# team-attention/nobs-whisper

Hardware: AMD Instinct MI355X
Metric: audio-sec/s (RTF⁻¹) large-v3 greedy, batch 128; 1/2/4/8 MI355X (higher is better)
Workload: dtype bf16

## Files before the change

### include/whisper_mi355x.h

```cpp
#ifndef WHISPER_MI355X_H
#define WHISPER_MI355X_H

#include "whisper.h"

#ifdef __cplusplus
extern "C" {
#endif

#define WHISPER_MI355X_ERR_RUNTIME (-10)

enum whisper_mi355x_dtype { WHISPER_MI355X_F16 = 0, WHISPER_MI355X_BF16 = 1, WHISPER_MI355X_FP8_ENC = 2 };

WHISPER_API struct whisper_context * whisper_mi355x_init(const char * path_model, struct whisper_context_params params,
                                                         int dtype, bool load_weights);

WHISPER_API int whisper_mi355x_weight_arena(struct whisper_context * ctx, void ** dev_ptr, size_t * bytes);

WHISPER_API int whisper_mi355x_rccl_unique_id(char out[128]);
WHISPER_API int whisper_mi355x_broadcast_weights(struct whisper_context * ctx, const char unique_id[128], int rank, int world);

WHISPER_API int whisper_mi355x_full_batch(struct whisper_context * ctx, struct whisper_state * state,
                                          struct whisper_full_params params, const float * const * pcm,
                                          const int * n_samples, int n_jobs, bool pcm_on_device, int fixed_tokens);
WHISPER_API int whisper_mi355x_full_batch_forced(struct whisper_context * ctx, struct whisper_state * state,
// ... 42 lines not shown

WHISPER_API int whisper_mi355x_kernel_timing(struct whisper_state * state, int class_mask);
WHISPER_API int whisper_mi355x_kernel_stats(struct whisper_state * state, int cls, double out[3]);
#define WHISPER_MI355X_KSTAT_PDEC_GIVE_UPS 100
WHISPER_API long whisper_mi355x_pdec_give_ups(struct whisper_state * state);
#define WHISPER_MI355X_KSTAT_BEAM_GATHER 101

WHISPER_API int whisper_mi355x_debug_gemm(struct whisper_context * ctx, int epi, const void * A, int M, int K,
                                          const void * B, int N, const float * bias, void * out, int reps, float * ms);
WHISPER_API void whisper_mi355x_set_gemm_variant(int variant);
WHISPER_API void whisper_mi355x_set_gemm_stamps(void * dev);
WHISPER_API int whisper_mi355x_debug_gemm_small(struct whisper_context * ctx, int epi, const void * A, int M, int K,
                                                const void * B, int N, const float * bias, void * out,
                                                const float * ln_w, const float * ln_b, int reps, float * ms);
WHISPER_API void whisper_mi355x_set_dec_splits(int splits);
WHISPER_API void whisper_mi355x_set_dec_bm(int rows);
WHISPER_API void whisper_mi355x_set_pdec_spin(long ticks);
WHISPER_API void whisper_mi355x_set_pdec_stamps(void * dev);
WHISPER_API void whisper_mi355x_set_pdec_blocks(int on);
WHISPER_API int whisper_mi355x_debug_gemm_fp8(struct whisper_context * ctx, int epi, const void * A8,
                                              const float * a_scale, int M, int K, const void * B8,
                                              const float * b_scale, int N, const float * bias, void * out,
                                              int reps, float * ms);
WHISPER_API int whisper_mi355x_debug_gemm_w8(struct whisper_context * ctx, int epi, const void * A, int M, int K,
                                             const void * B8, const float * b_scale, int N, const float * bias,
                                             void * out, const float * ln_w, const float * ln_b, void * y);
WHISPER_API int whisper_mi355x_debug_quant_fp8(struct whisper_context * ctx, const void * x, long rows, int K,
                                               void * q, float * s);
WHISPER_API int whisper_mi355x_debug_attn_encoder(struct whisper_context * ctx, const void * qkv, int B, int T, int d,
                                                  int H, int variant, void * out, int reps, float * ms);
WHISPER_API int whisper_mi355x_debug_gemm_ln(struct whisper_context * ctx, const void * A, int M, int K,
                                             const void * B, int N, const float * bias, float * x,
                                             const float * ln_w, const float * ln_b, void * y, int reps, float * ms);

WHISPER_API int whisper_mi355x_debug_xattn(struct whisper_context * ctx, const void * enc, const int * slot,
                                           const void * q, const void * wkt, const void * wv, const float * bv,
                                           int n, int n_ctx, int d, float scale, int splits, float rescale_thr,
                                           void * out, int reps, float * ms);

WHISPER_API int whisper_mi355x_debug_attn_self_step(struct whisper_context * ctx, const float * slabs, int splits,
                                                    const float * bias, float scale, void * cache, const int * slot,
                                                    const int * pos, int n, int L, int layer, int H, int n_ctx,
                                                    void * out);
WHISPER_API int whisper_mi355x_debug_attn_cross_step(struct whisper_context * ctx, const float * slabs, int splits,
                                                     const float * bias, float scale, const void * cache,
                                                     const int * slot, const int * n_kv, int n, int L, int layer,
                                                     int H, int n_ctx, void * out);
WHISPER_API int whisper_mi355x_debug_attn_prefill(struct whisper_context * ctx, const void * q, int q_stride,
                                                  const void * cache, const int * slot, const int * n_kv,
                                                  const void * tiles, int n_tiles, int L, int layer, int H, int n_ctx,
                                                  void * out);

struct whisper_mi355x_cand {
    int32_t id, tid;
    float   p, plog, pt, ptsum, no_speech_prob, pad;
};
WHISPER_API int whisper_mi355x_debug_logits_topk(struct whisper_context * ctx, const float * logits, int n,
                                                 const int * rules, const float * temperature, int k, int split,
                                                 struct whisper_mi355x_cand * cand, struct whisper_mi355x_cand * greedy);
WHISPER_API int whisper_mi355x_debug_kv_gather(struct whisper_context * ctx, void * cache, int n_slots, int L, int H,
                                               int n_ctx, const int * copies, int n_copies, int * n_staged);

struct whisper_mi355x_seq_ctl {
    int32_t is_initial, last_ts, penult_ts, has_ts, seek_delta;
    float   temperature;
    int32_t suppress_blank, no_timestamps, suppress_eot, tid0_initial;
// ... 46 lines not shown
```

### nobs-whisper_amd/csrc/capi.cpp

```cpp
#include <cmath>
#include <cstring>
#include <string>
#include <thread>
#include <vector>

#include <rccl/rccl.h>

#include "../../include/whisper_mi355x.h"
#include "engine.h"

namespace wm { extern int g_gemm_variant; extern int g_dec_splits; extern int g_dec_bm; extern unsigned long long* g_gemm_stamps; }
using namespace wm;

static Context* C(whisper_context* ctx) { return ctx ? &ctx->c : nullptr; }

template <typename F> static int guarded(whisper_state* s, F&& f) {
    try {
        return f();
    } catch (const wm::Error&) {
    } catch (const std::bad_alloc&) {
        fprintf(stderr, "whisper_mi355x: host out of memory\n");
    }
    if (s) recover_state(s);
    return WHISPER_MI355X_ERR_RUNTIME;
// ... 743 lines not shown
int whisper_mi355x_debug_gemm_ln(struct whisper_context* ctx, const void* A, int M, int K, const void* B, int N,
                                 const float* bias, float* x, const float* ln_w, const float* ln_b, void* y, int reps,
                                 float* ms) {
    return guarded(nullptr, [&]() -> int {
        if (!ctx || M > 128) return -1;
        hipSetDevice(ctx->c.device);
        hipStream_t st;
        WM_CHECK(hipStreamCreate(&st));
        GemmArgs g{};
        g.A = A; g.a_rpb = M; g.a_bstride = 0; g.a_rstride = K;
        g.B = B; g.bias = bias; g.M = M; g.N = N; g.K = K;
        g.out = x; g.ldo = N; g.o_rpb = M; g.o_bstride = 0; g.o_off = 0;
        g.sc_div = 0; g.sc_mod = 1; g.sc_lim = 0; g.scale = 1.0f;
        g.ln_w = ln_w; g.ln_b = ln_b; g.ln_out = y;
        g.splitk_ws_elems = 64L * M * N;
        WM_CHECK(hipMalloc(&g.splitk_ws, g.splitk_ws_elems * sizeof(float)));
        hipEvent_t e0, e1;
        WM_CHECK(hipEventCreate(&e0));
        WM_CHECK(hipEventCreate(&e1));
        WM_CHECK(hipEventRecord(e0, st));
        for (int r = 0; r < std::max(1, reps); r++) launch_gemm(ctx->c.dt, EPI_RESID, g, st);
        WM_CHECK(hipEventRecord(e1, st));
        WM_CHECK(hipStreamSynchronize(st));
        float t = 0;
        WM_CHECK(hipEventElapsedTime(&t, e0, e1));
        if (ms) *ms = t / std::max(1, reps);
        hipEventDestroy(e0);
        hipEventDestroy(e1);
        hipStreamDestroy(st);
        hipFree(g.splitk_ws);
        return 0;
    });
}
int whisper_mi355x_debug_xattn(struct whisper_context* ctx, const void* enc, const int* slot, const void* q,
                               const void* wkt, const void* wv, const float* bv, int n, int n_ctx, int d, float scale,
                               int splits, float rescale_thr, void* out, int reps, float* ms) {
    return guarded(nullptr, [&]() -> int {
        if (!ctx || n <= 0 || !xattn_supported(d)) return -1;
        hipSetDevice(ctx->c.device);
        const DType dt = ctx->c.dt;
        const int H = d / 64;
        if (splits <= 0) splits = xattn_splits(n, n_ctx);
        void* qx = nullptr;
        float *op = nullptr, *ml = nullptr;
        WM_CHECK(hipMalloc(&qx, (size_t)n * 2 * H * d * 2));
        WM_CHECK(hipMalloc((void**)&op, (size_t)n * splits * H * d * 4));
        WM_CHECK(hipMalloc((void**)&ml, (size_t)n * splits * H * 2 * 4));
        hipStream_t st;
        WM_CHECK(hipStreamCreate(&st));
        auto run = [&] {
            launch_xattn_qproj(dt, q, wkt, n, d, H, scale, qx, st);
            launch_xattn_step(dt, enc, slot, qx, n, n_ctx, d, splits, rescale_thr, op, ml, st);
            launch_xattn_combine(dt, op, ml, splits, wv, bv, n, d, H, out, st);
        };
        hipEvent_t e0, e1;
        WM_CHECK(hipEventCreate(&e0));
        WM_CHECK(hipEventCreate(&e1));
        run();
        WM_CHECK(hipEventRecord(e0, st));
        for (int r = 0; r < reps; r++) run();
        WM_CHECK(hipEventRecord(e1, st));
        WM_CHECK(hipStreamSynchronize(st));
        float t = 0;
        WM_CHECK(hipEventElapsedTime(&t, e0, e1));
        if (ms) *ms = reps > 0 ? t / reps : 0.0f;
        hipEventDestroy(e0);
// ... 330 lines not shown
```

### nobs-whisper_amd/csrc/engine.cpp

```cpp
#include <algorithm>
#include <chrono>
#include <cmath>
#include <cstring>
#include <exception>
#include <thread>

#include "engine.h"

namespace wm {

static size_t esize(DType) { return 2; }

static void dfree(void*& p) {
    if (p) { void* q = p; p = nullptr; WM_CHECK(hipFree(q)); }
}
template <typename T> static void dfree(T*& p) {
    void* q = (void*)p;
    p = nullptr;
    dfree(q);
}
template <typename T> static void dalloc(T*& p, size_t bytes) {
    void* q = nullptr;
    p = nullptr;
    WM_CHECK(hipMalloc(&q, bytes));
// ... 705 lines not shown
    w.n_qtiles = nt;
    WM_CHECK(hipMemcpyAsync(w.qtiles, w.h_qtiles, (size_t)nt * sizeof(int2), hipMemcpyHostToDevice, s->stream));
}

struct DecView {
    int r0, n;
    hipStream_t st;
    float* splitk;
    long splitk_elems;
    float *xo, *xml;
};

static int small_m_max() {
    const char* e = getenv("WHISPER_MI355X_SMALLM");
    if (!e) return 4;
    const int v = atoi(e);
    return v == 1 ? 32 : std::max(0, std::min(32, v));
}

static int quant_small_max() {
    const char* e = getenv("WHISPER_MI355X_QSMALL_MAX");
    return e ? atoi(e) : 32;
}

static int pdec_max() {
    const char* e = getenv("WHISPER_MI355X_PDEC");
    return e ? std::max(0, std::min(kPdecMaxRows, atoi(e))) : kPdecMaxRows;
}

static int small_rows_max(Context* c) { return c->quant ? std::max(quant_small_max(), small_m_max()) : small_m_max(); }

static bool dec_fp8(Context* c) { return c->fp8_enc && !c->dec8.empty(); }

static int dec_path_sig() {
    return small_m_max() | (std::min(std::max(quant_small_max(), 0), 1023) << 6) |
           (std::min(std::max(attn_cross_wide_max(), 0), 1023) << 16) | (pdec_max() << 26) | ((g_pdec_blocks & 1) << 29);
}

static bool pdec_blocks(Context* c) {
    return c->quant && (g_pdec_blocks || !c->expanded.load(std::memory_order_acquire));
}

static bool pdec_use(Context* c, whisper_state* s, int n, bool xdirect) {
    if (xdirect || s->pdec_off || s->split_slots || n < 1 || n > pdec_max()) return false;
    if (dec_fp8(c)) return false;
    const bool quant = c->w.dec[0].qqkv.type != 0;
    for (const LayerW& L : c->w.dec)
        for (const QMat* q : {&L.qqkv, &L.qo, &L.qxq, &L.qxo, &L.q1, &L.q2})
            if ((q->type != 0) != quant) return false;
    const bool blocks = pdec_blocks(c);
    if (blocks && c->dt != DType::F16) return false;
    if (!pdec_supported(c->hp.n_text_state, c->hp.n_text_head, blocks)) return false;
    static const int cus = [] {
        int dev = 0, v = 0;
        hipGetDevice(&dev);
        hipDeviceGetAttribute(&v, hipDeviceAttributeMultiprocessorCount, dev);
        return v;
    }();
    return cus == 256;
}

static int dec_groups(int n_tok) { return cdiv(n_tok, 128); }

enum StepPath { STEP_PDEC, STEP_SMALL, STEP_SPLITK };
struct StepPlan {
    int n;
    int groups, gsz;
    StepPath path, tail_path;
    bool xdirect;
// ... 207 lines not shown
    const Hparams& hp = c->hp;
    Workspace& w = s->ws;
    const int d = hp.n_text_state, H = hp.n_text_head, V = hp.n_vocab, L = hp.n_text_layer;
    const DType dt = c->dt;
    const Weights& W = c->w;
    hipStream_t st = v.st;
    const int n = v.n;
    const DecRows r = dec_rows(c, s, v);
    const int KCLS = K_GEMM_DEC;
    const double kvrow = (double)H * 64 * 2 * 2;
    const int kt_stride = kt_layer_stride(s);
    auto gemm = [&](int epi, const GemmArgs& g) { tgemm_ws(s, KCLS, dt, epi, g, st, v.splitk, v.splitk_elems); };
    auto use8 = [&](GemmArgs g, void* q8, float* sc) {
        if (P.w8) { g.B = q8; g.w8_scale = sc; }
        return g;
    };
    auto resid = [&](const void* A, int K, const void* Wt, const float* bias, const float* lnw, const float* lnb, void* q8,
                     float* sc) {
        GemmArgs g = use8(gemm_plain(A, n, K, Wt, d, bias, r.dx, d), q8, sc);
        g.ln_w = lnw; g.ln_b = lnb; g.ln_out = r.dh;
        gemm(EPI_RESID, g);
    };
    auto partials = [&](const void* A, const void* Wt, int N, const float* bias, float scale, void* q8,
                        float* sc) -> DecSlabs {
        GemmArgs g = use8(gemm_plain(A, n, d, Wt, N, bias, nullptr, N), q8, sc);
        g.splitk_ws = v.splitk;
        g.splitk_ws_elems = v.splitk_elems;
        g.slab_wt = 1;
        KT kt(s, KCLS, 2.0 * g.N * g.K + 2.0 * g.M * g.K + 4.0 * g.M * g.N, st);
        const int splits = launch_gemm_partials(dt, g, st);
        if (splits <= 0 || splits > 16) WM_FAIL("decode partials GEMM not applicable (splits %d)", splits);
        return DecSlabs{v.splitk, splits, (long)n * N, N, bias, scale};
    };
    embed_rows(c, r, true);
    for (int l = 0; l < L; l++) {
        const LayerW Lw = layer_dense(c, s, l, st);
        static const Context::Fp8Dec no8{};
        const Context::Fp8Dec& F = P.w8 ? c->dec8[l] : no8;
        const bool kt_layer = l % kt_stride == 0;
        {
            const DecSlabs sl = partials(r.dh, Lw.wqkv, 3 * d, Lw.bqkv, c->k_scale, F.wqkv, F.sqkv);
            KT kt(s, K_ATTN_SELF, self_share, st, kt_layer);
            launch_attn_self_step(dt, sl, w.self, r.sslot, r.pos, n, L, l, H, hp.n_text_ctx, d, r.datt, st);
        }
        resid(r.datt, d, Lw.wo, Lw.bo, Lw.lnx_w, Lw.lnx_b, F.wo, F.so);
        if (P.xdirect) {
            GemmArgs g = use8(gemm_plain(r.dh, n, d, Lw.wxq, d, Lw.bxq, r.dq, d), F.wxq, F.sxq);
            g.scale = c->k_scale; g.sc_div = d; g.sc_mod = 1; g.sc_lim = 1;
            gemm(EPI_STORE, g);
            xattn_tail(c, s, v, r, l, K_ATTN_CROSS, kt_layer);
        } else {
            const DecSlabs sl = partials(r.dh, Lw.wxq, d, Lw.bxq, c->k_scale, F.wxq, F.sxq);
            KT kt(s, K_ATTN_CROSS, (double)n * hp.n_audio_ctx * kvrow, st, kt_layer);
            launch_attn_cross_step(dt, sl, w.cross, r.slot, r.nkv_cross, n, L, l, H, hp.n_audio_ctx, d, r.datt, st);
        }
        resid(r.datt, d, Lw.wxo, Lw.bxo, Lw.ln2_w, Lw.ln2_b, F.wxo, F.sxo);
        gemm(EPI_GELU, use8(gemm_plain(r.dh, n, d, Lw.w1, 4 * d, Lw.b1, r.dff, 4 * d), F.w1, F.s1));
        if (l + 1 < L) resid(r.dff, 4 * d, Lw.w2, Lw.b2, W.dec[l + 1].ln1_w, W.dec[l + 1].ln1_b, F.w2, F.s2);
        else resid(r.dff, 4 * d, Lw.w2, Lw.b2, W.lnd_w, W.lnd_b, F.w2, F.s2);
    }
    gemm(EPI_F32, gemm_plain(r.dh, n, d, W.tok_emb, V, nullptr, w.logits + (size_t)v.r0 * V, V));
}

struct AlignPass {
    const AlignClip* clips;
    int n_clips, max_rows;
    long total_rows;
    float* P;
};
static void decoder_rows_prefill(Context* c, whisper_state* s, const DecView& v, int n_rows, bool xdirect,
                                 const AlignPass* al = nullptr) {
    const Hparams& hp = c->hp;
    Workspace& w = s->ws;
    const int d = hp.n_text_state, H = hp.n_text_head, V = hp.n_vocab, L = hp.n_text_layer;
    const DType dt = c->dt;
    const Weights& W = c->w;
    hipStream_t st = v.st;
    const int n = v.n;
    const DecRows r = dec_rows(c, s, v);
    const int KCLS = K_GEMM_DEC;
    const double kvrow = (double)H * 64 * 2 * 2;
    const int kt_stride = kt_layer_stride(s);
    auto gemm = [&](int epi, const GemmArgs& g) { tgemm_ws(s, KCLS, dt, epi, g, st, v.splitk, v.splitk_elems); };
    auto resid = [&](const void* A, int K, const void* Wt, const float* bias, const float* lnw, const float* lnb) {
        gemm(EPI_RESID, gemm_plain(A, n, K, Wt, d, bias, r.dx, d));
        if (lnw) launch_layernorm(dt, r.dx, nullptr, n, d, lnw, lnb, r.dh, st);
    };
    embed_rows(c, r, false);
    launch_layernorm(dt, r.dx, nullptr, n, d, W.dec[0].ln1_w, W.dec[0].ln1_b, r.dh, st);
    for (int l = 0; l < L; l++) {
// ... 656 lines not shown
        return;
    }
    WM_CHECK(hipMemcpyAsync(w.h_tout, w.tout, n * sizeof(TokOut), hipMemcpyDeviceToHost, st));
    probs_rows.assign(n, {});
    if (any_probs) {
        const size_t V = c->hp.n_vocab;
        for (int r = 0; r < n; r++)
            if (w.h_ctl[r].want_probs) {
                probs_rows[r].resize(2 * V);
                WM_CHECK(hipMemcpyAsync(probs_rows[r].data(), w.probs + (size_t)r * 2 * V, 2 * V * 4, hipMemcpyDeviceToHost, st));
            }
    }
    WM_CHECK(hipStreamSynchronize(st));
}
static void run_logits(Sched& S, const std::vector<int>& act, bool want_nosp, std::vector<std::vector<float>>& probs_rows) {
    const bool any = logits_prepare(S, act, want_nosp);
    logits_launch(S.c, S.s, (int)act.size());
    logits_finish(S, (int)act.size(), any, probs_rows);
}

static const double kPdecBackoffMs = 1000.0;

static const unsigned* pd_err_ptr(Context* c, whisper_state* s, int pd) {
    const Hparams& hp = c->hp;
    Workspace& w = s->ws;
    if (pd == 1) return (const unsigned*)((const char*)w.pd_sync + pdec_granules(hp.n_text_state, hp.n_text_layer, hp.n_text_head).err_bytes);
    return nullptr;
}
static size_t ring_slot_bytes(const Workspace& w) { return (size_t)w.cap_jobs * sizeof(TokOut) + 16; }

static whisper_state::DecGraph* dec_graph(Context* c, whisper_state* s, StepPlan P, int par) {
    const int n = P.n, pd = P.path == STEP_PDEC;
    P.pipe = par > 0;
    const int sig = dec_path_sig();
    const int beam = s->beam_k | (s->split_slots ? 1 << 8 : 0);
    const int gen = g_pdec_gen.load(std::memory_order_acquire);
    for (size_t i = 0; i < s->dec_graphs.size();) {
        auto& g = s->dec_graphs[i];
        if (g.pdec && g.gen != gen) {
            hipGraphExecDestroy(g.exec);
            for (auto& e : g.ev) { hipEventDestroy(e.a); hipEventDestroy(e.b); }
            s->dec_graphs.erase(s->dec_graphs.begin() + i);
        } else {
            i++;
        }
    }
    for (auto& g : s->dec_graphs)
        if (g.n_tok == n && g.n_rows == n && g.mask == s->ktime_mask && g.direct == s->direct && g.sig == sig && g.pdec == pd &&
            g.par == par && g.beam == beam)
            return &g;
    whisper_state::DecGraph g{n, n, s->ktime_mask, s->direct, sig, pd, gen, par, beam, nullptr, {}};
    hipGraph_t graph;
    s->capture_ev = &g.ev;
    WM_CHECK(hipStreamBeginCapture(s->stream, hipStreamCaptureModeThreadLocal));
    decoder_launch(c, s, P);
    logits_launch(c, s, n);
    if (par > 0) {
        Workspace& w = s->ws;
        char* slot = w.ring + (par - 1) * ring_slot_bytes(w);
        launch_decode_advance(n, w.cap_tok, c->vid.beg, w.tout, w.tok, w.ctl, (TokOut*)slot, pd_err_ptr(c, s, pd),
                              (unsigned*)(slot + (size_t)w.cap_jobs * sizeof(TokOut)), s->stream);
    }
    WM_CHECK(hipStreamEndCapture(s->stream, &graph));
    s->capture_ev = nullptr;
    WM_CHECK(hipGraphInstantiate(&g.exec, graph, nullptr, nullptr, 0));
    WM_CHECK(hipGraphDestroy(graph));
    s->dec_graphs.push_back(std::move(g));
// ... 786 lines not shown
```

### nobs-whisper_amd/csrc/engine.h

```cpp
#pragma once
#include <map>
#include <atomic>
#include <mutex>
#include <random>
#include <string>
#include <vector>

#include "../../include/whisper_mi355x.h"
#include "beam.h"
#include "common.h"
#include "kernels.h"

namespace wm {

struct Hparams {
    int32_t n_vocab, n_audio_ctx, n_audio_state, n_audio_head, n_audio_layer;
    int32_t n_text_ctx, n_text_state, n_text_head, n_text_layer, n_mels, ftype;
};

struct Vocab {
    int n_vocab = 51864;
    int token_eot = 50256, token_sot = 50257, token_translate = 50357, token_transcribe = 50358;
    int token_solm = 50359, token_prev = 50360, token_nosp = 50361, token_not = 50362, token_beg = 50363;
    std::map<std::string, int> token_to_id;
// ... 157 lines not shown
struct KStat { double ms = 0, work = 0; long count = 0; };

}

struct whisper_state {
    wm::Context* ctx = nullptr;
    int device = 0;
    hipStream_t stream = nullptr;
    hipStream_t stream2 = nullptr;
    hipEvent_t ev_fork = nullptr, ev_join = nullptr;
    wm::Workspace ws;
    bool direct = false;
    std::vector<std::vector<wm::Segment>> results;
    std::vector<int> lang_ids;
    std::vector<std::vector<whisper_mi355x_window_decision>> decisions;
    std::vector<int> prompt_past;
    std::mt19937 rng{0};
    int lang_id = 0;
    int n_len = 0, n_len_org = 0;
    std::vector<float> logits_host;
    double phase_ms[5] = {0, 0, 0, 0, 0};
    double align_ms = 0;
    struct AlignInfo { int rows = 0, frames = 0; const float* cost = nullptr; };
    std::vector<AlignInfo> align_info;
    long decoded_tokens = 0;
    int last_enc_windows = 0;
    bool mel_ready = false;
    bool pooled = false;
    int ktime_mask = 0;
    wm::KStat kstat[wm::K_NCLASS];
    struct KPending { int cls; hipEvent_t a, b; double work; };
    std::vector<KPending> kpending;
    std::vector<hipEvent_t> kpool;
    struct DecGraph { int n_tok, n_rows, mask; bool direct; int sig; int pdec; int gen; int par; int beam; hipGraphExec_t exec; std::vector<KPending> ev; };
    std::vector<DecGraph> dec_graphs;
    std::vector<KPending>* capture_ev = nullptr;
    double cur_self_work = 0;
    whisper_state* twin = nullptr;
    long pdec_give_ups = 0;
    double pdec_lost_ms = 0;
    double pdec_off_until = 0;
    bool pdec_off = false;
    int beam_k = 0;
    bool split_slots = false;
    struct BeamRec { std::vector<int> tokens; double sum_logprobs_all = 0; int flags = 0; };
    std::vector<std::vector<BeamRec>> beam_info;
    double gather_rows = 0, gather_rows_full = 0;
};

struct whisper_context {
    wm::Context c;
};

namespace wm {
bool load_context(Context* c, const char* path, int device, DType dt, bool load_weights);
void free_context(Context* c);
whisper_state* new_state(Context* c);
void free_state(whisper_state* s);
void recover_state(whisper_state* s);
void drain_state_pool(Context* c);
void orphan_states(Context* c);
bool resolve_dtw(Context* c, const whisper_context_params& cp);

struct FullOpts {
    int fixed_tokens = 0;
    const int* forced = nullptr;
    const int* spot = nullptr;
// ... 13 lines not shown
```

### nobs-whisper_amd/csrc/kernels.h

```cpp
#pragma once
#include <atomic>

#include "common.h"

namespace wm {

void launch_mel(const float* const* d_pcm, const int* d_n, const void* d_tab, const float* d_filt_t, int n_mel,
                float* const* d_mel, const int* d_nlen, int* d_max, int n_jobs, int max_frames, hipStream_t st);
void launch_mel_window(DType dt, float* const* d_mel, const int* d_nlen, const int* d_n, const int* d_max,
                       const int* d_win_job, const int* d_win_seek, int n_win, int n_mel, void* out, hipStream_t st);
void launch_mel_normalize(const float* d_mel, int nl, int n_samples, const int* d_max, int n_mel, float* out, hipStream_t st);
void launch_silence_boundaries(const float* const* pcm, const int* n_samples, int n_clips, int max_n, int sample_rate,
                               float* rms, int rms_stride, int* counts, int* bounds, int cap, float* floor_out,
                               hipStream_t st);
void launch_resample(const float* const* in, const int* n_in, int n_clips, int max_out, const float* W, int ldw, int fsi,
                     int fso, float* const* out, const int* n_out, hipStream_t st);

void launch_layernorm(DType dt, const float* x, const int* rows, int M, int D, const float* w, const float* b,
                      void* y, hipStream_t st);
void launch_embed(DType dt, const void* tok_emb, bool te_f32, const float* pos_emb, const int* tok, const int* pos,
                  int n, int D, float* x, hipStream_t st);
void launch_embed_ln(DType dt, const void* tok_emb, bool te_f32, const float* pos_emb, const int* tok, const int* pos,
                     int n, int D, float* x, const float* w, const float* b, void* y, hipStream_t st);

// ... 11 lines not shown
struct QMat {
    int type = 0;
    const uint8_t* qs = nullptr;
    const uint32_t* qh = nullptr;
    const uint16_t* dm = nullptr;
};

struct GemmArgs {
    const void* A; long a_rpb, a_bstride, a_rstride;
    const void* B;
    const float* bias;
    int M, N, K;
    void* out; long ldo; long o_rpb, o_bstride, o_off;
    const float* pos; int pos_rows;
    float scale; int sc_div, sc_mod, sc_lim;
    void* cache; const int* row_slot; const int* row_pos; int L, layer, H, ctx, d;
    float* splitk_ws; long splitk_ws_elems;
    const float* ln_w; const float* ln_b; void* ln_out;
    const float* a_ln_w; const float* a_ln_b;
    QMat q;
    int slab_wt;
    const float* w8_scale;
    unsigned long long* stamps;
};
extern unsigned long long* g_gemm_stamps;

void launch_gemm(DType dt, int epi, const GemmArgs& a, hipStream_t st);
void launch_gemm_fp8(DType dt, int epi, const GemmArgs& a, const float* a_scale, const float* b_scale, hipStream_t st);
void launch_quant_rows_fp8(DType dt, const void* x, long rows, int K, void* q, float* s, hipStream_t st);
void launch_layernorm_fp8(const float* x, int M, int D, const float* w, const float* b, void* q, float* s,
                          hipStream_t st);
void init_gelu_table();
int launch_gemm_partials(DType dt, const GemmArgs& a, hipStream_t st);
bool gemm_small_ok(int M, int K, bool lna);
void launch_dequant(DType dt, const QMat& q, long rows, int K, void* out, hipStream_t st);
struct DequantJobs {
    int n = 0;
    QMat q[6];
    long rows[6];
    int K[6];
    void* out[6];
    long start[7];
};
void launch_dequant_multi(DType dt, DequantJobs J, hipStream_t st);
void launch_gemm_small(DType dt, int epi, const GemmArgs& a, bool lna, hipStream_t st);

void launch_attn_encoder(DType dt, const void* qkv, void* out, int B, int T, int d, int H, hipStream_t st,
                         int variant = -1);
void launch_attn_prefill(DType dt, const void* q, int q_stride, const void* cache, const int* slot, const int* n_kv,
                         const void* tiles, int n_tiles, int L, int layer, int H, int ctx, int d, void* out,
                         hipStream_t st);

struct DecSlabs {
    const float* ws; int splits; long zstride; int ld; const float* bias; float scale;
};
void launch_attn_self_step(DType dt, const DecSlabs& sl, void* cache, const int* slot, const int* pos, int n, int L,
                           int layer, int H, int ctx, int d, void* out, hipStream_t st);
int attn_cross_wide_max();
void launch_attn_cross_step(DType dt, const DecSlabs& sl, const void* cache, const int* slot, const int* n_kv, int n,
                            int L, int layer, int H, int ctx, int d, void* out, hipStream_t st);

bool xattn_supported(int d);
int xattn_splits(int n, int Tn);
void launch_xattn_qproj(DType dt, const void* q, const void* wkt, int n, int d, int H, float scale, void* qx,
                        hipStream_t st);
void launch_xattn_step(DType dt, const void* enc, const int* slot, const void* qx, int n, int Tn, int d, int splits,
// ... 110 lines not shown
```

### nobs-whisper_amd/csrc/kernels/gemm.hip

```cpp
#include <mutex>
#include "../common.h"
#include "../kernels.h"

#include <algorithm>
#include <cmath>
#include <type_traits>
#include <vector>

namespace wm {

typedef uint32_t u32x4 __attribute__((ext_vector_type(4)));

__device__ uint16_t g_gelu_tab[65536];

void init_gelu_table() {
    static std::vector<uint16_t> tab;
    static std::mutex mu;
    std::lock_guard<std::mutex> lk(mu);
    if (tab.empty()) {
        tab.resize(65536);
        const float GELU_COEF_A = 0.044715f;
        const float SQRT_2_OVER_PI = 0.79788456080286535587989211986876f;
        for (int i = 0; i < 65536; i++) {
            const uint16_t u = (uint16_t)i;
// ... 1003 lines not shown
                const int row = wm * (BM / 2) + i * 16 + (lane & 15);
                af[i] = __builtin_bit_cast(FT, st[row * 8 + (ch ^ ((row >> 1) & 7))]);
            }
#pragma unroll
            for (int j = 0; j < 2; j++) {
                const int row = wn * 32 + j * 16 + (lane & 15);
                if constexpr (W8) {
                    const uint2 w8 = ((const uint2*)&st[BM * 8 + row * 4 + ((ch >> 1) ^ ((row >> 2) & 3))])[ch & 1];
                    uint32_t e[4];
                    if constexpr (std::is_same<T, half_t>::value) {
                        typedef _Float16 v2h __attribute__((ext_vector_type(2)));
                        e[0] = __builtin_bit_cast(uint32_t, (v2h)__builtin_amdgcn_cvt_scalef32_pk_f16_fp8(w8.x, 1.0f, false));
                        e[1] = __builtin_bit_cast(uint32_t, (v2h)__builtin_amdgcn_cvt_scalef32_pk_f16_fp8(w8.x, 1.0f, true));
                        e[2] = __builtin_bit_cast(uint32_t, (v2h)__builtin_amdgcn_cvt_scalef32_pk_f16_fp8(w8.y, 1.0f, false));
                        e[3] = __builtin_bit_cast(uint32_t, (v2h)__builtin_amdgcn_cvt_scalef32_pk_f16_fp8(w8.y, 1.0f, true));
                    } else {
                        typedef __bf16 v2b __attribute__((ext_vector_type(2)));
                        e[0] = __builtin_bit_cast(uint32_t, (v2b)__builtin_amdgcn_cvt_scalef32_pk_bf16_fp8(w8.x, 1.0f, false));
                        e[1] = __builtin_bit_cast(uint32_t, (v2b)__builtin_amdgcn_cvt_scalef32_pk_bf16_fp8(w8.x, 1.0f, true));
                        e[2] = __builtin_bit_cast(uint32_t, (v2b)__builtin_amdgcn_cvt_scalef32_pk_bf16_fp8(w8.y, 1.0f, false));
                        e[3] = __builtin_bit_cast(uint32_t, (v2b)__builtin_amdgcn_cvt_scalef32_pk_bf16_fp8(w8.y, 1.0f, true));
                    }
                    bfr[j] = __builtin_bit_cast(FT, e);
                } else {
                    bfr[j] = __builtin_bit_cast(FT, st[BM * 8 + row * 8 + (ch ^ ((row >> 1) & 7))]);
                }
            }
#pragma unroll
            for (int i = 0; i < MI; i++)
#pragma unroll
                for (int j = 0; j < 2; j++) acc[i][j] = mfma16x16x32(af[i], bfr[j], acc[i][j]);
        }
        if (t + MAXT < nkt) {
            __syncthreads();
            issue(t + MAXT);
        }
    }
#pragma unroll
    for (int i = 0; i < MI; i++)
#pragma unroll
        for (int j = 0; j < 2; j++) {
            const int n = n0 + wn * 32 + j * 16 + (lane & 15);
            if (n >= g.N) continue;
            const float wsc = W8 ? g.w8_scale[n] : 1.0f;
#pragma unroll
            for (int r = 0; r < 4; r++) {
                const int m = m0 + wm * (BM / 2) + i * 16 + (lane >> 4) * 4 + r;
                if (m >= g.M) continue;
                const float v = W8 ? acc[i][j][r] * wsc : acc[i][j][r];
                if constexpr (SPLIT) {
                    float* p = &g.splitk_ws[((long)blockIdx.z * g.M + m) * g.N + n];
                    if (g.slab_wt) __hip_atomic_store(p, v, __ATOMIC_RELAXED, __HIP_MEMORY_SCOPE_AGENT);
                    else *p = v;
                }
                else epilogue<EPI, T>(g, m, n, v);
            }
        }
}

int g_gemm_variant = -1;
unsigned long long* g_gemm_stamps = nullptr;

int g_dec_bm = 0;
static int dec_bm_min() {
    static const int v = getenv("WHISPER_MI355X_DEC_BM") ? atoi(getenv("WHISPER_MI355X_DEC_BM")) : 32;
    return g_dec_bm > 0 ? g_dec_bm : v;
}
// ... 430 lines not shown
        case EPI_GELU: launch_small_t<T, EPI_GELU>(g, lna, st); break;
        case EPI_RESID: launch_small_t<T, EPI_RESID>(g, lna, st); break;
        case EPI_F32: launch_small_t<T, EPI_F32>(g, lna, st); break;
        default: WM_FAIL("small-M GEMM epilogue %d not supported", epi);
    }
}

void launch_gemm_small(DType dt, int epi, const GemmArgs& g, bool lna, hipStream_t st) {
    if (g.M <= 0 || g.N <= 0) return;
    if (!gemm_small_ok(g.M, g.K, lna) || g.o_rpb != g.M || g.a_rpb != g.M || g.o_off || (epi == EPI_STORE && g.o_bstride))
        WM_FAIL("small-M GEMM shape not supported (M=%d K=%d)", g.M, g.K);
    if (dt == DType::F16) launch_small_dt<half_t>(epi, g, lna, st);
    else launch_small_dt<bf16_t>(epi, g, lna, st);
}

int g_dec_splits = 0;
static int dec_splits_override() { return g_dec_splits; }
static int dec_splits_for(int tiles, int nk) {
    int splits = 1;
    while (tiles * (splits + 1) <= 256 && splits < 12 && (splits + 1) * 2 <= nk) splits++;
    return splits;
}
struct DecPlan { int splits, kc; };
static DecPlan dec_plan(int N, int K, int M, long ws_elems) {
    const int nk = K / 64;
    int splits = dec_splits_for(cdiv(N, 64), nk);
    if (dec_splits_override() > 0) splits = std::min(dec_splits_override(), nk);
    const int kc = cdiv(nk, splits) * 64;
    splits = cdiv(K, kc);
    if ((long)splits * M * N > ws_elems) return {0, 0};
    return {splits, kc};
}

template <typename T>
static void launch_reduce_resid_ln(const GemmArgs& g, int splits, hipStream_t st, bool ln4 = true) {
    if (ln4 && g.N % 4 == 0 && g.N <= 4096 && splits <= 16) {
        const int threads = cdiv(g.N / 4, 64) * 64;
        splitk_reduce_resid_ln4_kernel<T><<<g.M, threads, 0, st>>>(g, splits);
        return;
    }
    const int npt = cdiv(g.N, 256);
    if (npt <= 4) splitk_reduce_resid_ln_kernel<T, 4><<<g.M, 256, 0, st>>>(g, splits);
    else if (npt <= 8) splitk_reduce_resid_ln_kernel<T, 8><<<g.M, 256, 0, st>>>(g, splits);
    else WM_FAIL("fused LN width %d > 2048", g.N);
}

template <typename T, int EPI>
static void launch_splitk_reduce(const GemmArgs& g, int splits, hipStream_t st) {
    const long total = (long)g.M * g.N, work = (g.N & 3) == 0 ? total / 4 : total;
    const int thr = work < 65536 ? 64 : 256;
    splitk_reduce_kernel<T, EPI><<<std::min<long>(4096, cdiv(work, thr)), thr, 0, st>>>(g, splits);
}

static int gemm_group_m(int tiles_n) {
    static const int env = getenv("WHISPER_MI355X_GEMM_GM") ? atoi(getenv("WHISPER_MI355X_GEMM_GM")) : -1;
    if (env >= 0) return env;
    return tiles_n >= 8 ? 4 : 0;
}

template <typename T, int EPI>
static void launch_t(const GemmArgs& g, hipStream_t st) {
    if (g.w8_scale) {
        const bool fused_ln = EPI == EPI_RESID && g.ln_out != nullptr;
        if (!(g.splitk_ws && g.M <= 128 && g.K % 64 == 0 && g_gemm_variant != 0 && (EPI != EPI_RESID || fused_ln))) WM_FAIL("e4m3 weights need the decode-step GEMM path (M %d <= 128, K %% 64 == 0)", g.M);
    }
    const bool big256 = g_gemm_variant >= 2 ||
// ... 138 lines not shown
```

Baseline: 3424.

## Add whole-K decoder GEMM kernel with fused LayerNorm prologue behind seam flags

Adds a whole-K small-M GEMM kernel for decoder steps. It keeps all of A in LDS and streams B through a multi-stage global-to-LDS pipeline. It can apply LayerNorm to the fp32 residual inside its prologue, which lets the attention-out/cross-q and cross-out/FC1 seams skip separate split-K reduce+LN launches. The path is gated by WHISPER_MI355X_DEC_WK seam bits and is off by default. Separately, the existing GEMM's inter-tile __syncthreads is replaced by an LDS-only wait plus barrier, so outstanding global loads are no longer drained there. The graph signature is widened to long to key on the new setting.

Measured after the change: 3441 (median of 6 runs). About the same (+0.5%).

```diff
diff --git a/include/whisper_mi355x.h b/include/whisper_mi355x.h
--- a/include/whisper_mi355x.h
+++ b/include/whisper_mi355x.h
@@ -98,6 +98,10 @@
 WHISPER_API int whisper_mi355x_debug_gemm_ln(struct whisper_context * ctx, const void * A, int M, int K,
                                              const void * B, int N, const float * bias, float * x,
                                              const float * ln_w, const float * ln_b, void * y, int reps, float * ms);
+WHISPER_API void whisper_mi355x_set_dec_wk(int v);
+WHISPER_API int whisper_mi355x_debug_gemm_wk(struct whisper_context * ctx, int epi, const void * A, int M, int K,
+                                             const void * B, int N, const float * bias, void * out,
+                                             const float * ln_w, const float * ln_b, int reps, float * ms);
 
 WHISPER_API int whisper_mi355x_debug_xattn(struct whisper_context * ctx, const void * enc, const int * slot,
                                            const void * q, const void * wkt, const void * wv, const float * bv,
diff --git a/nobs-whisper_amd/csrc/capi.cpp b/nobs-whisper_amd/csrc/capi.cpp
--- a/nobs-whisper_amd/csrc/capi.cpp
+++ b/nobs-whisper_amd/csrc/capi.cpp
@@ -799,6 +799,41 @@
         return 0;
     });
 }
+void whisper_mi355x_set_dec_wk(int v) { wm::g_dec_wk = v; }
+int whisper_mi355x_debug_gemm_wk(struct whisper_context* ctx, int epi, const void* A, int M, int K, const void* B, int N,
+                                 const float* bias, void* out, const float* ln_w, const float* ln_b, int reps, float* ms) {
+    return guarded(nullptr, [&]() -> int {
+        if (!ctx || !A || !B || !out || M < 1 || M > 128 || N < 1 || K < 1) return -1;
+        if (epi != EPI_STORE && epi != EPI_GELU && epi != EPI_RESID) return -1;
+        const bool lna = ln_w != nullptr;
+        if (lna && (!ln_b || epi == EPI_RESID)) return -1;
+        GemmArgs g{};
+        g.A = A; g.a_rpb = M; g.a_bstride = 0; g.a_rstride = K;
+        g.B = B; g.bias = bias; g.M = M; g.N = N; g.K = K;
+        g.out = out; g.ldo = N; g.o_rpb = M; g.o_bstride = 0; g.o_off = 0;
+        g.sc_div = 0; g.sc_mod = 1; g.sc_lim = 0; g.scale = 1.0f;
+        g.a_ln_w = ln_w; g.a_ln_b = ln_b;
+        g.splitk_ws_elems = 64L * M * N;
+        if (!gemm_wk_ok(epi, g, lna)) return -1;
+        hipSetDevice(ctx->c.device);
+        hipStream_t st;
+        WM_CHECK(hipStreamCreate(&st));
+        hipEvent_t e0, e1;
+        WM_CHECK(hipEventCreate(&e0));
+        WM_CHECK(hipEventCreate(&e1));
+        WM_CHECK(hipEventRecord(e0, st));
+        for (int r = 0; r < std::max(1, reps); r++) launch_gemm_wk(ctx->c.dt, epi, g, lna, st);
+        WM_CHECK(hipEventRecord(e1, st));
+        WM_CHECK(hipStreamSynchronize(st));
+        float t = 0;
+        WM_CHECK(hipEventElapsedTime(&t, e0, e1));
+        if (ms) *ms = t / std::max(1, reps);
+        hipEventDestroy(e0);
+        hipEventDestroy(e1);
+        hipStreamDestroy(st);
+        return 0;
+    });
+}
 int whisper_mi355x_debug_xattn(struct whisper_context* ctx, const void* enc, const int* slot, const void* q,
                                const void* wkt, const void* wv, const float* bv, int n, int n_ctx, int d, float scale,
                                int splits, float rescale_thr, void* out, int reps, float* ms) {
diff --git a/nobs-whisper_amd/csrc/engine.cpp b/nobs-whisper_amd/csrc/engine.cpp
--- a/nobs-whisper_amd/csrc/engine.cpp
+++ b/nobs-whisper_amd/csrc/engine.cpp
@@ -761,9 +761,10 @@
 
 static bool dec_fp8(Context* c) { return c->fp8_enc && !c->dec8.empty(); }
 
-static int dec_path_sig() {
-    return small_m_max() | (std::min(std::max(quant_small_max(), 0), 1023) << 6) |
-           (std::min(std::max(attn_cross_wide_max(), 0), 1023) << 16) | (pdec_max() << 26) | ((g_pdec_blocks & 1) << 29);
+static long dec_path_sig() {
+    return (long)small_m_max() | (std::min(std::max(quant_small_max(), 0), 1023) << 6) |
+           (std::min(std::max(attn_cross_wide_max(), 0), 1023) << 16) | (pdec_max() << 26) | ((g_pdec_blocks & 1) << 29) |
+           ((long)dec_wk_seams() << 32);
 }
 
 static bool pdec_blocks(Context* c) {
@@ -1037,6 +1038,20 @@
         if (splits <= 0 || splits > 16) WM_FAIL("decode partials GEMM not applicable (splits %d)", splits);
         return DecSlabs{v.splitk, splits, (long)n * N, N, bias, scale};
     };
+    const int wk = P.w8 ? 0 : dec_wk_seams();
+    auto wk_ok = [&](int epi, GemmArgs g, bool lna) {
+        g.splitk_ws_elems = v.splitk_elems;
+        return gemm_wk_ok(epi, g, lna);
+    };
+    auto gemm_wk = [&](int epi, GemmArgs g, bool lna) {
+        g.splitk_ws_elems = v.splitk_elems;
+        KT kt(s, KCLS, 2.0 * g.N * g.K + (lna ? 4.0 : 2.0) * g.M * g.K + 4.0 * g.M * g.N, st);
+        launch_gemm_wk(dt, epi, g, lna, st);
+    };
+    auto with_ln = [&](GemmArgs g, const float* lnw, const float* lnb) {
+        g.A = r.dx; g.a_rstride = d; g.a_ln_w = lnw; g.a_ln_b = lnb;
+        return g;
+    };
     embed_rows(c, r, true);
     for (int l = 0; l < L; l++) {
         const LayerW Lw = layer_dense(c, s, l, st);
@@ -1048,19 +1063,37 @@
             KT kt(s, K_ATTN_SELF, self_share, st, kt_layer);
             launch_attn_self_step(dt, sl, w.self, r.sslot, r.pos, n, L, l, H, hp.n_text_ctx, d, r.datt, st);
         }
-        resid(r.datt, d, Lw.wo, Lw.bo, Lw.lnx_w, Lw.lnx_b, F.wo, F.so);
+        GemmArgs gq = gemm_plain(r.dh, n, d, Lw.wxq, d, Lw.bxq, r.dq, d);
+        if (P.xdirect) { gq.scale = c->k_scale; gq.sc_div = d; gq.sc_mod = 1; gq.sc_lim = 1; }
+        else { gq.bias = nullptr; gq.out = v.splitk; }
+        const int epi_q = P.xdirect ? EPI_STORE : EPI_F32;
+        const bool q_fits = (long)n * d <= v.splitk_elems;
+        const GemmArgs go = gemm_plain(r.datt, n, d, Lw.wo, d, Lw.bo, r.dx, d);
+        const bool move_x = (wk & 4) && q_fits && wk_ok(EPI_RESID, go, false) && wk_ok(epi_q, with_ln(gq, Lw.lnx_w, Lw.lnx_b), true);
+        const bool wk_q = move_x || ((wk & 1) && q_fits && wk_ok(epi_q, gq, false));
+        if (move_x) gemm_wk(EPI_RESID, go, false);
+        else resid(r.datt, d, Lw.wo, Lw.bo, Lw.lnx_w, Lw.lnx_b, F.wo, F.so);
+        if (wk_q) gemm_wk(epi_q, move_x ? with_ln(gq, Lw.lnx_w, Lw.lnx_b) : gq, move_x);
         if (P.xdirect) {
-            GemmArgs g = use8(gemm_plain(r.dh, n, d, Lw.wxq, d, Lw.bxq, r.dq, d), F.wxq, F.sxq);
-            g.scale = c->k_scale; g.sc_div = d; g.sc_mod = 1; g.sc_lim = 1;
-            gemm(EPI_STORE, g);
+            if (!wk_q) gemm(EPI_STORE, use8(gq, F.wxq, F.sxq));
             xattn_tail(c, s, v, r, l, K_ATTN_CROSS, kt_layer);
         } else {
-            const DecSlabs sl = partials(r.dh, Lw.wxq, d, Lw.bxq, c->k_scale, F.wxq, F.sxq);
+            const DecSlabs sl = wk_q ? DecSlabs{v.splitk, 1, (long)n * d, d, Lw.bxq, c->k_scale}
+                                     : partials(r.dh, Lw.wxq, d, Lw.bxq, c->k_scale, F.wxq, F.sxq);
             KT kt(s, K_ATTN_CROSS, (double)n * hp.n_audio_ctx * kvrow, st, kt_layer);
             launch_attn_cross_step(dt, sl, w.cross, r.slot, r.nkv_cross, n, L, l, H, hp.n_audio_ctx, d, r.datt, st);
         }
-        resid(r.datt, d, Lw.wxo, Lw.bxo, Lw.ln2_w, Lw.ln2_b, F.wxo, F.sxo);
-        gemm(EPI_GELU, use8(gemm_plain(r.dh, n, d, Lw.w1, 4 * d, Lw.b1, r.dff, 4 * d), F.w1, F.s1));
+        const GemmArgs gxo = gemm_plain(r.datt, n, d, Lw.wxo, d, Lw.bxo, r.dx, d);
+        const GemmArgs g1 = gemm_plain(r.dh, n, d, Lw.w1, 4 * d, Lw.b1, r.dff, 4 * d);
+        const bool move_2 = (wk & 4) && wk_ok(EPI_RESID, gxo, false) && wk_ok(EPI_GELU, with_ln(g1, Lw.ln2_w, Lw.ln2_b), true);
+        if (move_2) {
+            gemm_wk(EPI_RESID, gxo, false);
+            gemm_wk(EPI_GELU, with_ln(g1, Lw.ln2_w, Lw.ln2_b), true);
+        } else {
+            resid(r.datt, d, Lw.wxo, Lw.bxo, Lw.ln2_w, Lw.ln2_b, F.wxo, F.sxo);
+            if ((wk & 2) && wk_ok(EPI_GELU, g1, false)) gemm_wk(EPI_GELU, g1, false);
+            else gemm(EPI_GELU, use8(g1, F.w1, F.s1));
+        }
         if (l + 1 < L) resid(r.dff, 4 * d, Lw.w2, Lw.b2, W.dec[l + 1].ln1_w, W.dec[l + 1].ln1_b, F.w2, F.s2);
         else resid(r.dff, 4 * d, Lw.w2, Lw.b2, W.lnd_w, W.lnd_b, F.w2, F.s2);
     }
@@ -1783,7 +1816,7 @@
 static whisper_state::DecGraph* dec_graph(Context* c, whisper_state* s, StepPlan P, int par) {
     const int n = P.n, pd = P.path == STEP_PDEC;
     P.pipe = par > 0;
-    const int sig = dec_path_sig();
+    const long sig = dec_path_sig();
     const int beam = s->beam_k | (s->split_slots ? 1 << 8 : 0);
     const int gen = g_pdec_gen.load(std::memory_order_acquire);
     for (size_t i = 0; i < s->dec_graphs.size();) {
diff --git a/nobs-whisper_amd/csrc/engine.h b/nobs-whisper_amd/csrc/engine.h
--- a/nobs-whisper_amd/csrc/engine.h
+++ b/nobs-whisper_amd/csrc/engine.h
@@ -213,7 +213,7 @@
     struct KPending { int cls; hipEvent_t a, b; double work; };
     std::vector<KPending> kpending;
     std::vector<hipEvent_t> kpool;
-    struct DecGraph { int n_tok, n_rows, mask; bool direct; int sig; int pdec; int gen; int par; int beam; hipGraphExec_t exec; std::vector<KPending> ev; };
+    struct DecGraph { int n_tok, n_rows, mask; bool direct; long sig; int pdec; int gen; int par; int beam; hipGraphExec_t exec; std::vector<KPending> ev; };
     std::vector<DecGraph> dec_graphs;
     std::vector<KPending>* capture_ev = nullptr;
     double cur_self_work = 0;
diff --git a/nobs-whisper_amd/csrc/kernels.h b/nobs-whisper_amd/csrc/kernels.h
--- a/nobs-whisper_amd/csrc/kernels.h
+++ b/nobs-whisper_amd/csrc/kernels.h
@@ -67,6 +67,10 @@
                           hipStream_t st);
 void init_gelu_table();
 int launch_gemm_partials(DType dt, const GemmArgs& a, hipStream_t st);
+extern int g_dec_wk;
+int dec_wk_seams();
+bool gemm_wk_ok(int epi, const GemmArgs& a, bool lna);
+void launch_gemm_wk(DType dt, int epi, const GemmArgs& a, bool lna, hipStream_t st);
 bool gemm_small_ok(int M, int K, bool lna);
 void launch_dequant(DType dt, const QMat& q, long rows, int K, void* out, hipStream_t st);
 struct DequantJobs {
diff --git a/nobs-whisper_amd/csrc/kernels/gemm.hip b/nobs-whisper_amd/csrc/kernels/gemm.hip
--- a/nobs-whisper_amd/csrc/kernels/gemm.hip
+++ b/nobs-whisper_amd/csrc/kernels/gemm.hip
@@ -1059,7 +1059,7 @@
                 for (int j = 0; j < 2; j++) acc[i][j] = mfma16x16x32(af[i], bfr[j], acc[i][j]);
         }
         if (t + MAXT < nkt) {
-            __syncthreads();
+            asm volatile("s_waitcnt lgkmcnt(0)\n\ts_barrier" ::: "memory");
             issue(t + MAXT);
         }
     }
@@ -1556,6 +1556,8 @@
     return {splits, kc};
 }
 
+#include "gemm_wk.h"
+
 template <typename T>
 static void launch_reduce_resid_ln(const GemmArgs& g, int splits, hipStream_t st, bool ln4 = true) {
     if (ln4 && g.N % 4 == 0 && g.N <= 4096 && splits <= 16) {
diff --git a/nobs-whisper_amd/csrc/kernels/gemm_wk.h b/nobs-whisper_amd/csrc/kernels/gemm_wk.h
--- /dev/null
+++ b/nobs-whisper_amd/csrc/kernels/gemm_wk.h
@@ -0,0 +1,225 @@
+
+__device__ __forceinline__ double wk_wave_sum(double v) {
+    v += __shfl_xor(v, 32);
+    v += __shfl_xor(v, 16);
+    v += dpp_f64<0x128>(v);
+    v += dpp_f64<0x124>(v);
+    v += dpp_f64<0x4E>(v);
+    v += dpp_f64<0xB1>(v);
+    return v;
+}
+
+__device__ __forceinline__ void wk_wait_barrier(int n) {
+#define WK_W(k) case k: asm volatile("s_waitcnt vmcnt(" #k ")\n\ts_barrier" ::: "memory"); break;
+    switch (n) {
+        WK_W(0) WK_W(1) WK_W(2) WK_W(3) WK_W(4) WK_W(5) WK_W(6) WK_W(7) WK_W(8) WK_W(9) WK_W(10) WK_W(11)
+        WK_W(12) WK_W(13) WK_W(14) WK_W(15) WK_W(16) WK_W(17) WK_W(18) WK_W(19) WK_W(20) WK_W(21) WK_W(22) WK_W(23)
+        WK_W(24) WK_W(25) WK_W(26) WK_W(27) WK_W(28) WK_W(29) WK_W(30) WK_W(31) WK_W(32) WK_W(33) WK_W(34) WK_W(35)
+        WK_W(36) WK_W(37) WK_W(38) WK_W(39) WK_W(40) WK_W(41) WK_W(42) WK_W(43) WK_W(44) WK_W(45) WK_W(46)
+        default: asm volatile("s_waitcnt vmcnt(47)\n\ts_barrier" ::: "memory"); break;
+    }
+#undef WK_W
+}
+
+template <typename T, int EPI, bool LNA>
+__global__ void __launch_bounds__(640) gemm_wk_kernel(const GemmArgs g, const int kc, const int S) {
+#pragma clang fp contract(off)
+    typedef typename Frag<T>::type FT;
+    typedef __attribute__((address_space(3))) void* lds_ptr_t;
+    extern __shared__ __attribute__((aligned(16))) char wk_smem[];
+    const int tid = threadIdx.x, lane = tid & 63, wave = tid >> 6, NW = blockDim.x >> 6;
+    const int BN = NW * 8;
+    const int wm = wave & 1, wn = wave >> 1;
+    const int n0 = blockIdx.x * BN, m0 = blockIdx.y * 32;
+    const int K = g.K, nkt = K / 64, kct = kc / 64;
+    u32x4* a_lds = (u32x4*)wk_smem;
+    u32x4* b_lds = a_lds + nkt * 256;
+    const int bstage = BN * 8;
+    const T* b_src;
+    {
+        const int r = wave * 8 + (lane >> 3);
+        const int c = (lane & 7) ^ ((r >> 1) & 7);
+        const int n = min(n0 + r, g.N - 1);
+        b_src = (const T*)g.B + (long)n * K + c * 8;
+    }
+    auto issue_b = [&](int t, int slot) {
+        __builtin_amdgcn_global_load_lds((const void*)(b_src + t * 64), (lds_ptr_t)&b_lds[slot * bstage + wave * 64], 16, 0, 2);
+    };
+    for (int t = 0; t < min(nkt, S); t++) issue_b(t, t);
+    if constexpr (!LNA) {
+        const T* A = (const T*)g.A;
+        for (int p = wave; p < nkt * 4; p += NW) {
+            const int r = (p & 3) * 8 + (lane >> 3);
+            const int c = (lane & 7) ^ ((r >> 1) & 7);
+            const int m = min(m0 + r, g.M - 1);
+            __builtin_amdgcn_global_load_lds((const void*)(A + (long)m * g.a_rstride + (p >> 2) * 64 + c * 8),
+                                             (lds_ptr_t)&a_lds[p * 64], 16, 0, 0);
+        }
+    } else {
+        const int nseg = (K + 255) >> 8;
+        for (int r0 = wave; r0 < 32; r0 += 4 * NW) {
+            float xa[4][5][4];
+#pragma unroll
+            for (int i = 0; i < 4; i++) {
+                const int m = min(m0 + min(r0 + i * NW, 31), g.M - 1);
+                const float* xr = (const float*)g.A + (long)m * g.a_rstride;
+#pragma unroll
+                for (int sg = 0; sg < 5; sg++) {
+                    const int n = sg * 256 + lane * 4;
+                    const float4 v = sg < nseg && n < K ? *(const float4*)(xr + n) : make_float4(0.f, 0.f, 0.f, 0.f);
+                    xa[i][sg][0] = v.x; xa[i][sg][1] = v.y; xa[i][sg][2] = v.z; xa[i][sg][3] = v.w;
+                }
+            }
+#pragma unroll
+            for (int i = 0; i < 4; i++) {
+                const int r = r0 + i * NW;
+                if (r >= 32) break;
+                float (&x)[5][4] = xa[i];
+                bool on[5];
+#pragma unroll
+                for (int sg = 0; sg < 5; sg++) on[sg] = sg < nseg && sg * 256 + lane * 4 < K;
+                double ws[5];
+#pragma unroll
+                for (int sg = 0; sg < 5; sg++)
+                    ws[sg] = wk_wave_sum(on[sg] ? (((double)x[sg][0] + (double)x[sg][1]) + (double)x[sg][2]) + (double)x[sg][3] : 0.0);
+                double s = 0.0;
+#pragma unroll
+                for (int sg = 0; sg < 5; sg++)
+                    if (sg < nseg) s += ws[sg];
+                const float mean = (float)(s / K);
+#pragma unroll
+                for (int sg = 0; sg < 5; sg++) {
+                    double s2 = 0.0;
+#pragma unroll
+                    for (int k = 0; k < 4; k++) {
+                        x[sg][k] = __fsub_rn(x[sg][k], mean);
+                        s2 += (double)__fmul_rn(x[sg][k], x[sg][k]);
+                    }
+                    ws[sg] = wk_wave_sum(on[sg] ? s2 : 0.0);
+                }
+                double q = 0.0;
+#pragma unroll
+                for (int sg = 0; sg < 5; sg++)
+                    if (sg < nseg) q += ws[sg];
+                const float variance = (float)(q / K);
+                const float scale = 1.0f / sqrtf(variance + 1e-5f);
+#pragma unroll
+                for (int sg = 0; sg < 5; sg++) {
+                    if (!on[sg]) continue;
+                    const int n = sg * 256 + lane * 4;
+                    const float4 w4 = *(const float4*)(g.a_ln_w + n), b4 = *(const float4*)(g.a_ln_b + n);
+                    const float wv[4] = {w4.x, w4.y, w4.z, w4.w}, bv[4] = {b4.x, b4.y, b4.z, b4.w};
+                    T y[4];
+#pragma unroll
+                    for (int k = 0; k < 4; k++) y[k] = (T)((x[sg][k] * scale) * wv[k] + bv[k]);
+                    const int ch = ((n >> 3) & 7) ^ ((r >> 1) & 7);
+                    *(uint2*)((char*)&a_lds[(n >> 6) * 256 + r * 8 + ch] + (n & 4) * 2) = *(const uint2*)y;
+                }
+            }
+        }
+    }
+    asm volatile("s_waitcnt vmcnt(0) lgkmcnt(0)\n\ts_barrier" ::: "memory");
+
+    f32x4 acc = {0.f, 0.f, 0.f, 0.f}, tot = {0.f, 0.f, 0.f, 0.f};
+    const int arow = wm * 16 + (lane & 15), brow = wn * 16 + (lane & 15);
+    const int asw = (arow >> 1) & 7, bsw = (brow >> 1) & 7;
+    int tc = 0, slot = 0;
+    for (int t = 0; t < nkt; t++) {
+        if (t > 0) wk_wait_barrier(min(nkt - 1, t + S - 1) - t);
+        const u32x4* at = a_lds + t * 256 + arow * 8;
+        const u32x4* bt = b_lds + slot * bstage + brow * 8;
+#pragma unroll
+        for (int s = 0; s < 2; s++) {
+            const int ch = s * 4 + (lane >> 4);
+            const FT af = __builtin_bit_cast(FT, at[ch ^ asw]);
+            const FT bf = __builtin_bit_cast(FT, bt[ch ^ bsw]);
+            acc = mfma16x16x32(af, bf, acc);
+        }
+        if (++tc == kct || t + 1 == nkt) {
+#pragma unroll
+            for (int r = 0; r < 4; r++) tot[r] = tot[r] + acc[r];
+            acc = (f32x4){0.f, 0.f, 0.f, 0.f};
+            tc = 0;
+        }
+        if (t + S < nkt) {
+            asm volatile("s_waitcnt lgkmcnt(0)\n\ts_barrier" ::: "memory");
+            issue_b(t + S, slot);
+        }
+        slot = slot + 1 == S ? 0 : slot + 1;
+    }
+    const int n = n0 + wn * 16 + (lane & 15);
+    if (n >= g.N) return;
+#pragma unroll
+    for (int r = 0; r < 4; r++) {
+        const int m = m0 + wm * 16 + (lane >> 4) * 4 + r;
+        if (m < g.M) epilogue<EPI, T>(g, m, n, tot[r]);
+    }
+}
+
+int g_dec_wk = -1;
+constexpr int kDecWkDefault = 0;
+int dec_wk_seams() {
+    static const int env = getenv("WHISPER_MI355X_DEC_WK") ? atoi(getenv("WHISPER_MI355X_DEC_WK")) : 1;
+    const int v = g_dec_wk >= 0 ? g_dec_wk : env;
+    return v <= 0 ? 0 : v == 1 ? kDecWkDefault : (v - 2) & 7;
+}
+
+static int wk_bn(int M, int N) {
+    static const int cand[4] = {32, 48, 64, 80};
+    const int rb = cdiv(M, 32);
+    for (int bn : cand)
+        if (cdiv(N, bn) % 8 == 0 && cdiv(N, bn) * rb <= 256) return bn;
+    for (int bn : cand)
+        if (cdiv(N, bn) * rb <= 256) return bn;
+    return 80;
+}
+
+bool gemm_wk_ok(int epi, const GemmArgs& g, bool lna) {
+    if (epi != EPI_STORE && epi != EPI_GELU && epi != EPI_RESID && epi != EPI_F32) return false;
+    if (g.M < 1 || g.M > 128 || g.N < 1 || g.K < 64 || g.K > 1280 || g.K % 64 != 0) return false;
+    if (g.w8_scale || g.q.type != 0 || g.a_rpb < g.M || !g.A || !g.B || !g.out) return false;
+    if (lna ? (!g.a_ln_w || !g.a_ln_b || g.a_rstride % 4 != 0 || ((uintptr_t)g.A & 15))
+            : (g.a_rstride % 8 != 0 || ((uintptr_t)g.A & 15)))
+        return false;
+    if (((uintptr_t)g.B & 15)) return false;
+    if (lna && (((uintptr_t)g.a_ln_w | (uintptr_t)g.a_ln_b) & 15)) return false;
+    return dec_plan(g.N, g.K, g.M, g.splitk_ws_elems).splits >= 2;
+}
+
+template <typename T, int EPI>
+static void launch_wk_t(const GemmArgs& g, bool lna, hipStream_t st) {
+    const DecPlan p = dec_plan(g.N, g.K, g.M, g.splitk_ws_elems);
+    const int bn = wk_bn(g.M, g.N), nkt = g.K / 64;
+    const size_t a_bytes = (size_t)nkt * 4096, stage = (size_t)bn * 128;
+    const int S = (int)std::max<size_t>(2, std::min<size_t>(std::min(16, nkt), (156 * 1024 - a_bytes) / stage));
+    const size_t smem = a_bytes + S * stage;
+    const dim3 grid(cdiv(g.N, bn), cdiv(g.M, 32));
+    if (lna) {
+        if constexpr (EPI == EPI_STORE || EPI == EPI_GELU || EPI == EPI_F32) {
+            static const bool attr = [] {
+                WM_CHECK(hipFuncSetAttribute((const void*)gemm_wk_kernel<T, EPI, true>, hipFuncAttributeMaxDynamicSharedMemorySize, 160 * 1024));
+                return true;
+            }();
+            gemm_wk_kernel<T, EPI, true><<<grid, bn * 8, smem, st>>>(g, p.kc, S);
+        } else {
+            WM_FAIL("whole-K GEMM: LayerNorm prologue with epilogue %d not supported", EPI);
+        }
+    } else {
+        static const bool attr = [] {
+            WM_CHECK(hipFuncSetAttribute((const void*)gemm_wk_kernel<T, EPI, false>, hipFuncAttributeMaxDynamicSharedMemorySize, 160 * 1024));
+            return true;
+        }();
+        gemm_wk_kernel<T, EPI, false><<<grid, bn * 8, smem, st>>>(g, p.kc, S);
+    }
+}
+
+void launch_gemm_wk(DType dt, int epi, const GemmArgs& g, bool lna, hipStream_t st) {
+    if (!gemm_wk_ok(epi, g, lna)) WM_FAIL("whole-K GEMM shape not supported (M=%d N=%d K=%d epi=%d)", g.M, g.N, g.K, epi);
+    const bool h = dt == DType::F16;
+    switch (epi) {
+        case EPI_STORE: h ? launch_wk_t<half_t, EPI_STORE>(g, lna, st) : launch_wk_t<bf16_t, EPI_STORE>(g, lna, st); break;
+        case EPI_GELU: h ? launch_wk_t<half_t, EPI_GELU>(g, lna, st) : launch_wk_t<bf16_t, EPI_GELU>(g, lna, st); break;
+        case EPI_RESID: h ? launch_wk_t<half_t, EPI_RESID>(g, lna, st) : launch_wk_t<bf16_t, EPI_RESID>(g, lna, st); break;
+        default: h ? launch_wk_t<half_t, EPI_F32>(g, lna, st) : launch_wk_t<bf16_t, EPI_F32>(g, lna, st); break;
+    }
+}
```
